# davlee1972/upscale_video

Hardware: AMD Instinct MI355X
Metric: frames/sec 1080p->2x Compact (SRVGGNetCompact per-frame SR hot path) (higher is better)
Workload: dtype f16 operands / f32 accumulate; 1 GPU; 2x_compact_1080p; tile_size=960, frames_per_call=1

## Files before the change

upscale_video_amd/csrc/uva_wino.hip.h:

```cpp
#pragma once
#include <type_traits>

#include "uva_devutil.hip.h"
#include "uva_wino.h"

namespace uva {

constexpr int TW_AROWB = 4 * 2 * 16 * 64;
constexpr int TW_BROWB = 4 * 2 * 15 * 64;
constexpr int TW_AROWS = 6, TW_BROWS = 10;
constexpr int TW_RAWROWB = 34 * 128;
constexpr int TW_RAWSLOTB = 4 * TW_RAWROWB;
constexpr int TW_RAW_PIECES = TW_RAWSLOTB / 1024;
constexpr int TW_ARING = 0;
constexpr int TW_BRING = TW_ARING + TW_AROWS * TW_AROWB;
constexpr int TW_RAW = TW_BRING + TW_BROWS * TW_BROWB;
constexpr int TW_PRM = TW_RAW + 2 * TW_RAWSLOTB;
constexpr int TW_FLAGS_OFF = TW_PRM + 2 * PARAM_LDS + 64;
constexpr int TW_LDS_BYTES = TW_FLAGS_OFF + 16;
static_assert(TW_RAW_PIECES == 17 && TW_RAWSLOTB % 1024 == 0, "raw slot = whole LDS-DMA pieces");
static_assert(TW_LDS_BYTES <= 160 * 1024, "trunkw kernel LDS budget");
static_assert(TW_RAW % 128 == 0 && TW_RAWROWB % 128 == 0, "raw pixel records are 128-byte aligned (the octet XOR flips address bits 4..6)");


__device__ __forceinline__ unsigned tw_piece_const(int i, int wave, int lane)
{
    const int q = (4 * i + wave) * 64 + lane;
    const int r = q / 272, u = q - r * 272;
    const int rec = u >> 3, sl = u & 7;
    const int par = rec >= 17 ? 1 : 0, h = rec - 17 * par;
    return (unsigned)((r << 13) | ((2 * h + par) * 128 + ((sl ^ (h & 7)) << 4)));
}

__device__ __forceinline__ unsigned dpp_row_shl1(unsigned v)
{
    return (unsigned)__builtin_amdgcn_mov_dpp((int)v, 0x101, 0xf, 0xf, true);
}
__device__ __forceinline__ unsigned pk_add_f16(unsigned a, unsigned b)
{
    return __builtin_bit_cast(unsigned, (half2v)(__builtin_bit_cast(half2v, a) + __builtin_bit_cast(half2v, b)));
}

#define TW_PRIO_K 2
#define TW_PRIO_E 0
#define TW_PRIO_KA TW_PRIO_K
#define TW_PRIO_EA TW_PRIO_E
#define TW_PRIO_KB TW_PRIO_K
#define TW_PRIO_EB TW_PRIO_E

#ifdef UVA_INSTRUMENT
#define TW_STAMP(k) do { if (stamp) a.dbg[16 * it + 8 * grp + (k)] = __builtin_amdgcn_s_memtime(); } while (0)
#else
#define TW_STAMP(k) do { } while (0)
#endif

template <int NF, int ACT>
__global__ __launch_bounds__(512, 2) UVA_NO_PK_F32 void trunkw_kernel(TrunkwArgs a)
{
    static_assert(NF == 64, "written for 64 features");
    constexpr int PIXB = 128;
    constexpr int TW_PFF = 12;
    constexpr int TW_PFF_B = 6;
    constexpr int TW_RAW_F0 = 4, TW_RAW_GAP = 12, TW_RAW_STRIDE = 3;
    constexpr int TW_DMA_PIECES = 5;
    constexpr int PFF_A = TW_PFF;

    extern __shared__ __attribute__((aligned(16))) char smem[];
    const unsigned lds0 = lds_offset(smem);
    float* const prm_all = (float*)(smem + TW_PRM);

    const int wave8 = __builtin_amdgcn_readfirstlane(threadIdx.x >> 6);
    const int grp = wave8 >> 2;
    const int wave = wave8 & 3;
    const int lane = threadIdx.x & 63;

#ifdef UVA_INSTRUMENT
    const unsigned long long t_entry = __builtin_amdgcn_s_memtime();
#endif
    const Trunk2Step* const steps = a.steps + (size_t)blockIdx.x * (a.max_steps + TW_PAD_STEPS);
    auto load_a = [&](int g) __attribute__((always_inline)) { return scalar_load16(&steps[g].a); };
    auto load_b = [&](int g) __attribute__((always_inline)) { return scalar_load16(&steps[g].b); };
    const uint4 e_first = load_a(0), e_second = load_a(1);
    const int nsteps = __builtin_amdgcn_readfirstlane(a.nsteps[blockIdx.x]);
    if (nsteps <= 0) return;
#ifdef UVA_INSTRUMENT
    const bool stamp = a.dbg != nullptr && blockIdx.x == 0 && (threadIdx.x & 255) == 0;
    if (stamp && grp == 0) a.dbg[16 * (nsteps + 2)] = t_entry;
#endif

    float prm_b = 0.f, prm_s = 0.f;
    if (wave == 0) {
        prm_b = (grp ? a.bias[1] : a.bias[0])[lane];
        prm_s = (grp ? a.slope[1] : a.slope[0])[lane];
    }
    half8 w[24];
    {
        const half8* wp = (const half8*)(grp ? a.wpk[1] : a.wpk[0]);
#pragma unroll
        for (int i = 0; i < 24; ++i) w[i] = wp[(i * 4 + wave) * 64 + lane];
    }
    unsigned dma_pc2[3];
#pragma unroll
    for (int i = 0; i < 3; ++i)
        dma_pc2[i] = tw_piece_const(2 * i, wave, lane) | (2 * i + 1 < 5 ? tw_piece_const(2 * i + 1, wave, lane) << 16 : 0u);
    auto issue_rows = [&](const uint4 e, int slot, auto i0c, auto i1c) __attribute__((always_inline)) {
        constexpr int I0 = decltype(i0c)::value, I1 = decltype(i1c)::value;
        const unsigned ey = __builtin_amdgcn_readfirstlane(e.y);
        const unsigned lo = __builtin_amdgcn_readfirstlane(e.x), hi = ey & 0xffu;
        const char* base = a.in_act + (((unsigned long long)hi << 32) | lo);
        const int pitch = __builtin_amdgcn_readfirstlane(e.z) & 0xffffff;
        const unsigned fadd = ((ey >> 27) & 1u) ? (unsigned)__builtin_amdgcn_readfirstlane(e.w) : 0u;
#pragma unroll
        for (int i = I0; i < I1; ++i) {
            if (4 * i + wave >= TW_RAW_PIECES) continue;
            const unsigned pc = (dma_pc2[i >> 1] >> (16 * (i & 1))) & 0xffffu;
            unsigned off = __umul24(pc >> 13, (unsigned)pitch) + (pc & 0x1fffu);
            if (fadd) off += (pc & 0x1800u) ? fadd : 0u;
            glds16_s(base, off, lds0 + TW_RAW + slot * TW_RAWSLOTB + (4 * i + wave) * 1024);
        }
    };

    auto vlane_of = [](int l) __attribute__((always_inline)) { const int p_ = l & 15, o_ = l >> 4; return (unsigned)(p_ * 64 + ((o_ ^ ((p_ >> 1) & 3)) << 4)); };

    const unsigned vlane_c = vlane_of(lane);
    const unsigned t_lo = (unsigned)((lane & 15) * PIXB + (((lane >> 4) ^ (lane & 7)) << 4));
    const unsigned t_hi = (unsigned)(((lane & 15) + 1) * PIXB + (((lane >> 4) ^ (((lane & 15) + 1) & 7)) << 4));
    auto transform_row = [&](const char* rrow, int pos) __attribute__((always_inline)) {
        const unsigned a_lo = t_lo, a_hi = t_hi;
        char* const vrow = smem + TW_ARING + pos * TW_AROWB + vlane_c;
        half8 d[2][4];
#pragma unroll
        for (int t = 0; t < 2; ++t) {
            d[t][0] = *(const half8*)(rrow + (a_lo ^ (t ? 64u : 0u)));
            d[t][1] = *(const half8*)(rrow + (a_lo ^ (t ? 64u : 0u)) + 17 * PIXB);
            d[t][2] = *(const half8*)(rrow + (a_hi ^ (t ? 64u : 0u)));
            d[t][3] = *(const half8*)(rrow + (a_hi ^ (t ? 64u : 0u)) + 17 * PIXB);
        }
#pragma unroll
        for (int t = 0; t < 2; ++t) {
            *(half8*)(vrow + 0 * 2048 + t * 1024) = pk_sub(d[t][0], d[t][2]);
            *(half8*)(vrow + 1 * 2048 + t * 1024) = d[t][1] + d[t][2];
            *(half8*)(vrow + 2 * 2048 + t * 1024) = pk_sub(d[t][2], d[t][1]);
            *(half8*)(vrow + 3 * 2048 + t * 1024) = pk_sub(d[t][1], d[t][3]);
        }
    };

    auto transform_half = [&](const char* rrow, int pos, int t) __attribute__((always_inline)) {
        const unsigned a_lo = t_lo ^ (t ? 64u : 0u), a_hi = t_hi ^ (t ? 64u : 0u);
        char* const vrow = smem + TW_ARING + pos * TW_AROWB + vlane_c + t * 1024;
        const half8 d0 = *(const half8*)(rrow + a_lo), d1 = *(const half8*)(rrow + a_lo + 17 * PIXB);
        const half8 d2 = *(const half8*)(rrow + a_hi), d3 = *(const half8*)(rrow + a_hi + 17 * PIXB);
        *(half8*)(vrow + 0 * 2048) = pk_sub(d0, d2);
        *(half8*)(vrow + 1 * 2048) = d1 + d2;
        *(half8*)(vrow + 2 * 2048) = pk_sub(d2, d1);
        *(half8*)(vrow + 3 * 2048) = pk_sub(d1, d3);
    };

    auto transform_rows = [&](int slot, int pos0) __attribute__((always_inline)) {
        int pos = pos0 + wave;
        pos = pos >= TW_AROWS ? pos - TW_AROWS : pos;
        transform_row(smem + TW_RAW + slot * TW_RAWSLOTB + wave * TW_RAWROWB, pos);
    };

    const bool six = (__builtin_amdgcn_readfirstlane(e_first.y) >> 25) & 1u;
    if (grp == 0) {
        issue_rows(e_first, 0, std::integral_constant<int, 0>{}, std::integral_constant<int, 5>{});
        issue_rows(e_second, 1, std::integral_constant<int, 0>{}, std::integral_constant<int, 5>{});
        if (six && wave < 2) {
            const unsigned lo = __builtin_amdgcn_readfirstlane(e_first.x), hi = __builtin_amdgcn_readfirstlane(e_first.y) & 0xffu;
            const int pitch = __builtin_amdgcn_readfirstlane(e_first.z) & 0xffffff;
            const char* base = a.in_act + (((unsigned long long)hi << 32) | lo) - (size_t)(2 - wave) * pitch;
#pragma unroll
            for (int i = 0; i < 5; ++i) {
                int q = i * 64 + lane;
                q = q < 272 ? q : 271;
                const int rec = q >> 3, sl = q & 7, par = rec >= 17 ? 1 : 0, hh = rec - 17 * par;
                glds16_s(base, (unsigned)((2 * hh + par) * 128 + ((sl ^ (hh & 7)) << 4)), lds0 + TW_BRING + wave * 5120 + i * 1024);
            }
        }
#pragma unroll
        for (int i = 0; i < 24; ++i) asm volatile("" : "+v"(w[i]));
        asm volatile("s_waitcnt vmcnt(0)" ::: "memory");
    }
    if (wave == 0) {
        float* prm = prm_all + grp * (PARAM_LDS / 4);
        prm[lane] = prm_b;
        prm[64 + lane] = prm_s;
        prm[128 + lane] = prm_s <= 1.f ? __builtin_inff() : -__builtin_inff();
    }
    group_barrier();
    if (grp == 1) {
        transform_rows(0, 2);
        if (six && wave < 2) transform_row(smem + TW_BRING + wave * 5120, wave);
    }
    group_barrier();

    const float* const bias_lds = prm_all + grp * (PARAM_LDS / 4);
    const float* const prm_lds = bias_lds + 64;
    const f32x4 zero4 = {0.f, 0.f, 0.f, 0.f};
    const f32x4 bias4 = *(const f32x4*)(bias_lds + 16 * wave + 4 * (lane >> 4));
    const f32x4 s4 = *(const f32x4*)(prm_lds + 16 * wave + 4 * (lane >> 4));
    const f32x4 i4 = *(const f32x4*)(prm_lds + 64 + 16 * wave + 4 * (lane >> 4));

    f32x4 acc[4][4];
    [[maybe_unused]] auto prefetch = [&](auto ring_tag, int base_pos, auto& pre) __attribute__((always_inline)) {
        constexpr bool BR = decltype(ring_tag)::value;
        constexpr int ROWB = BR ? TW_BROWB : TW_AROWB;
        constexpr int PFF = BR ? TW_PFF_B : PFF_A;
        static_assert(PFF <= 8, "the fragments read ahead of the barrier are window row 0's");
        const unsigned r0 = vlane_c + (unsigned)((BR ? TW_BRING : TW_ARING) + base_pos * ROWB);
#pragma unroll
        for (int f = 0; f < PFF; ++f) pre[f] = *(const half8*)(smem + r0 + (f & 3) * (ROWB / 4) + ((f >> 2) & 1) * (ROWB / 8));
    };
    auto kloop = [&](auto ring_tag, int base_pos, auto&& slice, auto&& hook, [[maybe_unused]] const auto& pre) __attribute__((always_inline)) {
        constexpr bool BR = decltype(ring_tag)::value;
        constexpr int INR = 0;
        constexpr int ROWB = BR ? TW_BROWB : TW_AROWB, NROWS = BR ? TW_BROWS : TW_AROWS;
        constexpr int JS = ROWB / 4, CS = ROWB / 8;
        constexpr int PFF = BR ? TW_PFF_B : PFF_A;
        constexpr int NFRAG = 48, RQ = PFF + 1;
        unsigned radr[6];
        const unsigned vlane = vlane_c;
#pragma unroll
        for (int R = 0; R < 6; ++R) {
            int pos = base_pos + R;
            pos = pos >= NROWS ? pos - NROWS : pos;
            radr[R] = vlane + (unsigned)((BR ? TW_BRING : TW_ARING) + pos * ROWB);
        }
        auto read_f = [&](int f) __attribute__((always_inline)) -> half8 {
            const int R = f >> 3, ch = (f >> 2) & 1, j = f & 3;
            return *(const half8*)(smem + radr[R] + j * JS + ch * CS);
        };
        half8 bq[RQ];
        __builtin_amdgcn_sched_barrier(0);
#pragma unroll
        for (int f = 0; f < PFF; ++f) {
            if constexpr (BR) bq[f] = pre[f];
            else bq[f] = read_f(f);
        }
        __builtin_amdgcn_sched_barrier(0);
        static_for<NFRAG>([&](auto fc) __attribute__((always_inline)) {
            constexpr int f = decltype(fc)::value;
            if constexpr (f + PFF < NFRAG) bq[(f + PFF) % RQ] = read_f(f + PFF);
            constexpr int R = f >> 3, ch = (f >> 2) & 1, j = f & 3;
            const half8 b = bq[f % RQ];
            static_for<4>([&](auto nc) __attribute__((always_inline)) {
                constexpr int n = decltype(nc)::value, dy = R - n;
                if constexpr (dy >= 0 && dy <= 2) {
                    constexpr bool first = dy == 0 && ch == 0;
                    acc[n][j] = __builtin_amdgcn_mfma_f32_16x16x32_f16(w[(j * 3 + dy) * 2 + ch], b, first ? (j == 1 ? bias4 : zero4) : acc[n][j], 0, 0, 0);
                }
            });
            if constexpr (R >= 3 && R - 3 < INR) slice(std::integral_constant<int, R - 3>{}, std::integral_constant<int, (f & 7)>{});
            hook(fc);
            __builtin_amdgcn_sched_barrier(0);
        });
    };

    struct RowSt {
        f32x2 u, v;
        unsigned x0, x1, y0, y1;
        unsigned t[4], q[8];
    };
    f32x2 neg1 = {-1.f, -1.f};
    asm volatile("" : "+v"(neg1));
    auto fin_sum = [&](RowSt& st, int n, int hh) __attribute__((always_inline)) {
        const f32x2 m0 = {acc[n][0][2 * hh], acc[n][0][2 * hh + 1]}, m1 = {acc[n][1][2 * hh], acc[n][1][2 * hh + 1]};
        const f32x2 m2 = {acc[n][2][2 * hh], acc[n][2][2 * hh + 1]}, m3 = {acc[n][3][2 * hh], acc[n][3][2 * hh + 1]};
        st.u = (m0 + m1) + m2;
        st.v = __builtin_elementwise_fma(m3, neg1, __builtin_elementwise_fma(m2, neg1, m1));
    };
    const half2v s16v[2] = {half2v{(_Float16)s4[0], (_Float16)s4[1]}, half2v{(_Float16)s4[2], (_Float16)s4[3]}};
    auto fin_act = [&](RowSt& st, int hh) __attribute__((always_inline)) {
        if constexpr (ACT != TW_ACT_F32) {
            const half2v hu = __builtin_convertvector(st.u, half2v), hv = __builtin_convertvector(st.v, half2v);
            const half2v mu = hu * s16v[hh], mv = hv * s16v[hh];
            const unsigned xu = __builtin_bit_cast(unsigned, __builtin_elementwise_max(hu, mu));
            const unsigned xv = __builtin_bit_cast(unsigned, __builtin_elementwise_max(hv, mv));
            if (hh == 0) { st.x0 = xu; st.y0 = xv; } else { st.x1 = xu; st.y1 = xv; }
            return;
        }
        const f32x2 sl = {s4[2 * hh], s4[2 * hh + 1]};
        const f32x2 us = st.u * sl, vs = st.v * sl;
        const f32x2 pu = {__builtin_amdgcn_fmed3f(st.u[0], us[0], i4[2 * hh]), __builtin_amdgcn_fmed3f(st.u[1], us[1], i4[2 * hh + 1])};
        const f32x2 pv = {__builtin_amdgcn_fmed3f(st.v[0], vs[0], i4[2 * hh]), __builtin_amdgcn_fmed3f(st.v[1], vs[1], i4[2 * hh + 1])};
        const unsigned xu = __builtin_bit_cast(unsigned, __builtin_convertvector(pu, half2v));
        const unsigned xv = __builtin_bit_cast(unsigned, __builtin_convertvector(pv, half2v));
        if (hh == 0) { st.x0 = xu; st.y0 = xv; } else { st.x1 = xu; st.y1 = xv; }
    };

    const int niter = nsteps + 2;
    __builtin_amdgcn_s_waitcnt(0x0f70);
    RowSt st2[2];
    if (grp == 0) {
        uint4 e_own = load_a(0);
        int a6 = 0;
        int b10 = 0;
        const int cg = lane >> 4, p = lane & 15;
        const int oo = 2 * (wave & 1) + (cg >> 1);
        const unsigned wlane = p < 15 ? (unsigned)(TW_BRING + (2 * (cg & 1)) * (TW_BROWB / 4) + (wave >> 1) * (TW_BROWB / 8) + p * 64 +
                                                    ((oo ^ ((p >> 1) & 3)) << 4))
                                      : (unsigned)(TW_FLAGS_OFF - 64 + 16 * cg);
        const unsigned w64 = (unsigned)(TW_BRING + (wave >> 1) * (TW_BROWB / 8) + p * 64 + ((oo ^ ((p >> 1) & 3)) << 4) + 8 * (cg & 1));
        const unsigned wrow = p < 15 ? (unsigned)TW_BROWB : 0u;
        const unsigned wj = p < 15 ? (unsigned)(TW_BROWB / 4) : 0u;
        half8 pre[PFF_A];
        for (int it = 0; it < niter; ++it) {
            TW_STAMP(0);
            const unsigned ey = __builtin_amdgcn_readfirstlane(e_own.y);
            int rmask = 15, b10w = b10;
            bool in0 = true, in1 = true, edge = false;
            auto set_step = [&](const unsigned eyv, const int b10v) __attribute__((always_inline)) {
                const int c_lo = (eyv >> 12) & 63, c_hi = (eyv >> 18) & 63;
                rmask = (eyv >> 8) & 15;
                const int pm = ((eyv >> 27) & 1u) ? (p & 7) : p;
                in0 = 2 * pm >= c_lo && 2 * pm < c_hi;
                in1 = 2 * pm + 1 >= c_lo && 2 * pm + 1 < c_hi;
                edge = rmask != 15 || c_lo != 0 || c_hi != 32;
                b10w = b10v;
            };
            auto slice = [&](RowSt& st, auto edge_tag, auto nc, auto kc) __attribute__((always_inline)) {
                constexpr int n = decltype(nc)::value, k = decltype(kc)::value;
                if constexpr (k == 0) fin_sum(st, n, 0);
                else if constexpr (k == 1) fin_act(st, 0);
                else if constexpr (k == 2) fin_sum(st, n, 1);
                else if constexpr (k == 3) fin_act(st, 1);
                else if constexpr (k == 4) {
                    if constexpr (decltype(edge_tag)::value) {
                        const bool rin = (rmask >> n) & 1;
                        const unsigned k0 = (rin && in0) ? 0xffffffffu : 0u, k1 = (rin && in1) ? 0xffffffffu : 0u;
                        st.x0 &= k0; st.x1 &= k0;
                        st.y0 &= k1; st.y1 &= k1;
                    }
                    st.t[0] = dpp_row_shl1(st.x0); st.t[1] = dpp_row_shl1(st.x1);
                    st.t[2] = dpp_row_shl1(st.y0); st.t[3] = dpp_row_shl1(st.y1);
                } else if constexpr (k == 5) {
                    st.q[0] = pk_sub_f16(st.x0, st.t[0]); st.q[1] = pk_sub_f16(st.x1, st.t[1]);
                    st.q[2] = pk_add_f16(st.y0, st.t[0]); st.q[3] = pk_add_f16(st.y1, st.t[1]);
                    st.q[4] = pk_sub_f16(st.t[0], st.y0); st.q[5] = pk_sub_f16(st.t[1], st.y1);
                    st.q[6] = pk_sub_f16(st.y0, st.t[2]); st.q[7] = pk_sub_f16(st.y1, st.t[3]);
                } else if constexpr (k == 6) {
                    int pos = b10w + n;
                    pos = pos >= TW_BROWS ? pos - TW_BROWS : pos;
                    if (p < 15) {
                        char* const w0 = smem + w64 + (unsigned)pos * TW_BROWB;
#pragma unroll
                        for (int j = 0; j < 4; ++j) *(uint2*)(w0 + j * (TW_BROWB / 4)) = make_uint2(st.q[2 * j], st.q[2 * j + 1]);
                    }
                } else if constexpr (k == 7) {
                } else if constexpr (k == 8) {
                    const auto s02a = __builtin_amdgcn_permlane16_swap(st.q[0], st.q[4], false, false);
                    const auto s02b = __builtin_amdgcn_permlane16_swap(st.q[1], st.q[5], false, false);
                    const auto s13a = __builtin_amdgcn_permlane16_swap(st.q[2], st.q[6], false, false);
                    const auto s13b = __builtin_amdgcn_permlane16_swap(st.q[3], st.q[7], false, false);
                    st.q[0] = s02a[0]; st.q[1] = s02b[0]; st.q[2] = s02a[1]; st.q[3] = s02b[1];
                    st.q[4] = s13a[0]; st.q[5] = s13b[0]; st.q[6] = s13a[1]; st.q[7] = s13b[1];
                } else {
                    int pos = b10w + n;
                    pos = pos >= TW_BROWS ? pos - TW_BROWS : pos;
                    char* const w0 = smem + wlane + (unsigned)pos * wrow;
                    *(uint4*)w0 = make_uint4(st.q[0], st.q[1], st.q[2], st.q[3]);
                    *(uint4*)(w0 + wj) = make_uint4(st.q[4], st.q[5], st.q[6], st.q[7]);
                }
            };
            set_step(ey, b10);
            if (it < nsteps) {
                __builtin_amdgcn_s_setprio(TW_PRIO_KA);
                auto no_hook = [](auto) __attribute__((always_inline)) {};
                kloop(std::false_type{}, a6, [&](auto nc, auto kc) __attribute__((always_inline)) { slice(st2[0], std::false_type{}, nc, kc); }, no_hook, pre);
                __builtin_amdgcn_s_setprio(TW_PRIO_EA);
            }
            TW_STAMP(1);
            group_barrier();
            TW_STAMP(2);
            if (it < nsteps) {
                auto rest = [&](auto edge_tag) __attribute__((always_inline)) {
                    static_for<2>([&](auto rc) __attribute__((always_inline)) {
                        static_for<8>([&](auto kc) __attribute__((always_inline)) {
                            slice(st2[0], edge_tag, std::integral_constant<int, 2 * decltype(rc)::value>{}, kc);
                            slice(st2[1], edge_tag, std::integral_constant<int, 2 * decltype(rc)::value + 1>{}, kc);
                        });
                    });
                };
                if (edge) rest(std::true_type{}); else rest(std::false_type{});
            }
            e_own = load_a(it + 1 < nsteps ? it + 1 : nsteps - 1);
            TW_STAMP(3);
            a6 = a6 + 4 >= TW_AROWS ? a6 + 4 - TW_AROWS : a6 + 4;
            group_barrier();
            b10 = b10 + 4 >= TW_BROWS ? b10 + 4 - TW_BROWS : b10 + 4;
        }
    } else {
        int a6 = 0, b10 = 0;
        uint4 e_k = make_uint4(0, 0, 0, 0), e_3 = make_uint4(0, 0, 0, 0);
        const int cg = lane >> 4, p = lane & 15;
        const int col = 2 * p + (cg & 1);
        const unsigned olane = (unsigned)(col * PIXB + 32 * wave + 16 * (cg >> 1));
        char* const sink = (char*)a.sink + lane * PIXB;
        const unsigned flip0 = (s4[0] > 1.f ? 0x8000u : 0u) | (s4[1] > 1.f ? 0x80000000u : 0u);
        const unsigned flip1 = (s4[2] > 1.f ? 0x8000u : 0u) | (s4[3] > 1.f ? 0x80000000u : 0u);
        auto make_slice = [&](const uint4 e) __attribute__((always_inline)) {
            const unsigned ey = __builtin_amdgcn_readfirstlane(e.y), lo = __builtin_amdgcn_readfirstlane(e.x);
            const size_t off = ((unsigned long long)(ey & 0xffu) << 32) | lo;
            const int pitch = __builtin_amdgcn_readfirstlane(e.z) & 0xffffff;
            const int vy = (ey >> 8) & 7, vx = (ey >> 11) & 63, v0 = (ey >> 17) & 7;
            const bool fold = (ey >> 25) & 1u;
            const unsigned fadd = fold ? (unsigned)__builtin_amdgcn_readfirstlane(e.w) : 0u;
            char* const obase = a.out_act + off + olane + ((fold && p >= 8) ? fadd : 0u);
            const bool colok = (fold ? (col & 15) : col) < vx;
            return [&, obase, pitch, vy, v0, colok](RowSt& st, auto nc, auto kc) __attribute__((always_inline)) {
                constexpr int n = decltype(nc)::value, k = decltype(kc)::value;
                if constexpr (k == 0) fin_sum(st, n, 0);
                else if constexpr (k == 1) fin_act(st, 0);
                else if constexpr (k == 2) fin_sum(st, n, 1);
                else if constexpr (k == 3) fin_act(st, 1);
                else if constexpr (k == 4) {
                    if constexpr (ACT == TW_ACT_F16_FLIP) {
                        st.x0 ^= flip0; st.y0 ^= flip0;
                        st.x1 ^= flip1; st.y1 ^= flip1;
                    }
                    const auto x = __builtin_amdgcn_permlane16_swap(st.x0, st.y0, false, false);
                    const auto y = __builtin_amdgcn_permlane16_swap(st.x1, st.y1, false, false);
                    st.q[0] = x[0]; st.q[1] = y[0]; st.q[2] = x[1]; st.q[3] = y[1];
                } else if constexpr (k == 5) {
                    char* dst = (n >= v0 && n < vy && colok) ? obase + (size_t)n * pitch : sink;
                    *(uint4*)dst = make_uint4(st.q[0], st.q[1], st.q[2], st.q[3]);
                }
            };
        };
        uint4 e_dma = load_a(2 <= nsteps + TW_PAD_STEPS - 1 ? 2 : nsteps + TW_PAD_STEPS - 1);
        unsigned st_prev = 0;
        for (int it = 0; it < niter; ++it) {
            TW_STAMP(0);
            issue_rows(e_dma, it & 1, std::integral_constant<int, 0>{}, std::integral_constant<int, TW_DMA_PIECES>{});
            e_dma = load_a(it + 3 <= nsteps + TW_PAD_STEPS - 1 ? it + 3 : nsteps + TW_PAD_STEPS - 1);
            const unsigned st_cur = (unsigned)__builtin_amdgcn_readfirstlane((int)(it >= 2 ? (__builtin_amdgcn_readfirstlane(e_3.y) >> 24) & 1u : 0u));
            if (it >= 2 && ((__builtin_amdgcn_readfirstlane(e_3.y) >> 24) & 1u)) {
                auto sl3 = make_slice(e_3);
                static_for<2>([&](auto rc) __attribute__((always_inline)) {
                    static_for<6>([&](auto kc) __attribute__((always_inline)) {
                        sl3(st2[0], std::integral_constant<int, 2 * decltype(rc)::value>{}, kc);
                        sl3(st2[1], std::integral_constant<int, 2 * decltype(rc)::value + 1>{}, kc);
                    });
                });
            }
            e_k = load_b(it >= 1 ? it - 1 : 0);
            const unsigned kact = (it >= 1 && it <= nsteps) ? (__builtin_amdgcn_readfirstlane(e_k.y) >> 24) & 1u : 0u;
            int bp = b10 - 4 - 2;
            bp = bp < 0 ? bp + TW_BROWS : bp;
            half8 pre[TW_PFF_B];
            TW_STAMP(1);
#ifdef UVA_INSTRUMENT
            asm volatile("s_waitcnt vmcnt(0)" ::: "memory");
            st_prev = st_cur;
#else
            {
                constexpr int P0 = TW_DMA_PIECES, P = TW_DMA_PIECES - 1;
                const unsigned nst = st_prev + st_cur;
                if (wave == 0) {
                    if (nst == 2) asm volatile("s_waitcnt vmcnt(%0)" ::"n"(P0 + 8) : "memory");
                    else if (nst == 1) asm volatile("s_waitcnt vmcnt(%0)" ::"n"(P0 + 4) : "memory");
                    else asm volatile("s_waitcnt vmcnt(%0)" ::"n"(P0) : "memory");
                } else {
                    if (nst == 2) asm volatile("s_waitcnt vmcnt(%0)" ::"n"(P + 8) : "memory");
                    else if (nst == 1) asm volatile("s_waitcnt vmcnt(%0)" ::"n"(P + 4) : "memory");
                    else asm volatile("s_waitcnt vmcnt(%0)" ::"n"(P) : "memory");
                }
                st_prev = st_cur;
            }
#endif
            prefetch(std::true_type{}, bp, pre);
            asm volatile("s_barrier" ::: "memory");
            TW_STAMP(2);
            [[maybe_unused]] auto raw_rows = [&]() __attribute__((always_inline)) {
                if (it + 1 < nsteps) {
                    int pos0 = a6 + 4 + 2;
                    pos0 = pos0 >= TW_AROWS ? pos0 - TW_AROWS : pos0;
                    transform_rows((it + 1) & 1, pos0);
                }
            };
            unsigned solo = (unsigned)__builtin_amdgcn_readfirstlane((int)((kact ^ 1u) & (it + 1 < nsteps ? 1u : 0u)));
            asm volatile("" : "+s"(solo));
            if (solo) {
                int pos = a6 + 4 + 2 + wave;
                pos = pos >= 2 * TW_AROWS ? pos - 2 * TW_AROWS : pos >= TW_AROWS ? pos - TW_AROWS : pos;
                const char* const rr = smem + TW_RAW + ((it + 1) & 1) * TW_RAWSLOTB + wave * TW_RAWROWB;
                transform_half(rr, pos, 0);
                __builtin_amdgcn_sched_barrier(0);
                transform_half(rr, pos, 1);
            }
            TW_STAMP(4);
            if (kact) {
                __builtin_amdgcn_s_setprio(TW_PRIO_KB);
                auto slk = make_slice(e_k);
                int rpos = a6 + 4 + 2 + wave;
                rpos = rpos >= 2 * TW_AROWS ? rpos - 2 * TW_AROWS : rpos >= TW_AROWS ? rpos - TW_AROWS : rpos;
                const char* const rrow = smem + TW_RAW + ((it + 1) & 1) * TW_RAWSLOTB + wave * TW_RAWROWB;
                char* const vrow = smem + TW_ARING + rpos * TW_AROWB + vlane_c;
                half8 rd[4];
                auto raw_hook = [&](auto fc) __attribute__((always_inline)) {
                    constexpr int f = decltype(fc)::value;
                    constexpr int H1 = TW_RAW_F0 + TW_RAW_GAP + 3 * TW_RAW_STRIDE + 1;
                    static_assert(H1 + TW_RAW_GAP + 3 * TW_RAW_STRIDE < 48, "the transform ends inside the k-loop");
                    constexpr int t = f >= H1 ? 1 : 0, g = f - (t ? H1 : TW_RAW_F0);
                    const unsigned a_lo = t_lo ^ (t ? 64u : 0u), a_hi = t_hi ^ (t ? 64u : 0u);
                    if constexpr (g == 0) {
                        rd[0] = *(const half8*)(rrow + a_lo); rd[1] = *(const half8*)(rrow + a_lo + 17 * PIXB);
                        rd[2] = *(const half8*)(rrow + a_hi); rd[3] = *(const half8*)(rrow + a_hi + 17 * PIXB);
                    } else if constexpr (g == TW_RAW_GAP) *(half8*)(vrow + 0 * 2048 + t * 1024) = pk_sub(rd[0], rd[2]);
                    else if constexpr (g == TW_RAW_GAP + TW_RAW_STRIDE) *(half8*)(vrow + 3 * 2048 + t * 1024) = pk_sub(rd[1], rd[3]);
                    else if constexpr (g == TW_RAW_GAP + 2 * TW_RAW_STRIDE) *(half8*)(vrow + 1 * 2048 + t * 1024) = rd[1] + rd[2];
                    else if constexpr (g == TW_RAW_GAP + 3 * TW_RAW_STRIDE) *(half8*)(vrow + 2 * 2048 + t * 1024) = pk_sub(rd[2], rd[1]);
                };
                kloop(std::true_type{}, bp, [&](auto nc, auto kc) __attribute__((always_inline)) { slk(st2[0], nc, kc); }, raw_hook, pre);
                __builtin_amdgcn_s_setprio(TW_PRIO_EB);
            }
            e_3 = e_k;
            TW_STAMP(3);
            group_barrier();
            a6 = a6 + 4 >= TW_AROWS ? a6 + 4 - TW_AROWS : a6 + 4;
            b10 = b10 + 4 >= TW_BROWS ? b10 + 4 - TW_BROWS : b10 + 4;
        }
    }
    asm volatile("s_waitcnt vmcnt(0)" ::: "memory");
}

}
```

Measured before the change: 493.4 frames/s.

## Carry partial row accumulators across Winograd k-loop iterations to skip recomputing overlap rows

Adds a carry mode in which the MFMA contributions from the last two input rows of each 6-row window are kept in extra accumulator registers (car) and reused as the starting value for the next iteration's first output rows. The k-loop then reads and multiplies only four new rows per step instead of six, and the prefetch depth and raw-transform schedule shrink to match. Slope, epilogue and DMA-offset constants are rematerialized per iteration instead of being held live, to offset the register pressure of the carry accumulators. The carried state adds a prologue kloop_carry pass and raises accumulator register use, which could hurt occupancy or the scheduling at 2 blocks per CU.

Result: no change. 497.0 frames/s (median of 6 runs) (+0.7%).

```diff
diff --git a/upscale_video_amd/csrc/uva_wino.hip.h b/upscale_video_amd/csrc/uva_wino.hip.h
--- a/upscale_video_amd/csrc/uva_wino.hip.h
+++ b/upscale_video_amd/csrc/uva_wino.hip.h
@@ -59,9 +59,26 @@
 {
     static_assert(NF == 64, "written for 64 features");
     constexpr int PIXB = 128;
-    constexpr int TW_PFF = 12;
-    constexpr int TW_PFF_B = 6;
-    constexpr int TW_RAW_F0 = 4, TW_RAW_GAP = 12, TW_RAW_STRIDE = 3;
+#ifndef TW_CARRY
+#define TW_CARRY 1
+#endif
+#ifndef TW_CARRY_GROUPS
+#define TW_CARRY_GROUPS 3
+#endif
+    constexpr bool CARRY_A = (TW_CARRY != 0) && (TW_CARRY_GROUPS & 1) != 0, CARRY_B = (TW_CARRY != 0) && (TW_CARRY_GROUPS & 2) != 0;
+#ifndef TW_PFF_A_
+#define TW_PFF_A_ (CARRY_A ? 8 : 12)
+#endif
+#ifndef TW_PFF_B_
+#define TW_PFF_B_ (CARRY_B ? 4 : 6)
+#endif
+#ifndef TW_RAW_SCHED
+#define TW_RAW_SCHED 1, 5, 2
+#endif
+    constexpr int TW_PFF = TW_PFF_A_;
+    constexpr int TW_PFF_B = TW_PFF_B_;
+    constexpr int raw_sched_[3] = {TW_RAW_SCHED};
+    constexpr int TW_RAW_F0 = CARRY_B ? raw_sched_[0] : 4, TW_RAW_GAP = CARRY_B ? raw_sched_[1] : 12, TW_RAW_STRIDE = CARRY_B ? raw_sched_[2] : 3;
     constexpr int TW_DMA_PIECES = 5;
     constexpr int PFF_A = TW_PFF;
 
@@ -103,21 +120,30 @@
 #pragma unroll
     for (int i = 0; i < 3; ++i)
         dma_pc2[i] = tw_piece_const(2 * i, wave, lane) | (2 * i + 1 < 5 ? tw_piece_const(2 * i + 1, wave, lane) << 16 : 0u);
-    auto issue_rows = [&](const uint4 e, int slot, auto i0c, auto i1c) __attribute__((always_inline)) {
+    auto piece_of = [&](int i, unsigned& row, unsigned& offs) __attribute__((always_inline)) {
+        const unsigned pc = (dma_pc2[i >> 1] >> (16 * (i & 1))) & 0xffffu;
+        row = pc >> 13;
+        offs = pc & 0x1fffu;
+    };
+    auto issue_rows = [&](const uint4 e, int slot, auto i0c, auto i1c, auto&& piece) __attribute__((always_inline)) {
         constexpr int I0 = decltype(i0c)::value, I1 = decltype(i1c)::value;
         const unsigned ey = __builtin_amdgcn_readfirstlane(e.y);
         const unsigned lo = __builtin_amdgcn_readfirstlane(e.x), hi = ey & 0xffu;
         const char* base = a.in_act + (((unsigned long long)hi << 32) | lo);
         const int pitch = __builtin_amdgcn_readfirstlane(e.z) & 0xffffff;
         const unsigned fadd = ((ey >> 27) & 1u) ? (unsigned)__builtin_amdgcn_readfirstlane(e.w) : 0u;
-#pragma unroll
-        for (int i = I0; i < I1; ++i) {
-            if (4 * i + wave >= TW_RAW_PIECES) continue;
-            const unsigned pc = (dma_pc2[i >> 1] >> (16 * (i & 1))) & 0xffffu;
-            unsigned off = __umul24(pc >> 13, (unsigned)pitch) + (pc & 0x1fffu);
-            if (fadd) off += (pc & 0x1800u) ? fadd : 0u;
-            glds16_s(base, off, lds0 + TW_RAW + slot * TW_RAWSLOTB + (4 * i + wave) * 1024);
-        }
+        auto pieces = [&](auto fold_tag) __attribute__((always_inline)) {
+#pragma unroll
+            for (int i = I0; i < I1; ++i) {
+                if (4 * i + wave >= TW_RAW_PIECES) continue;
+                unsigned row, offs;
+                piece(i, row, offs);
+                unsigned off = __umul24(row, (unsigned)pitch) + offs;
+                if constexpr (decltype(fold_tag)::value) off += (offs & 0x1800u) ? fadd : 0u;
+                glds16_s(base, off, lds0 + TW_RAW + slot * TW_RAWSLOTB + (4 * i + wave) * 1024);
+            }
+        };
+        if (fadd) pieces(std::true_type{}); else pieces(std::false_type{});
     };
 
     auto vlane_of = [](int l) __attribute__((always_inline)) { const int p_ = l & 15, o_ = l >> 4; return (unsigned)(p_ * 64 + ((o_ ^ ((p_ >> 1) & 3)) << 4)); };
@@ -164,8 +190,8 @@
 
     const bool six = (__builtin_amdgcn_readfirstlane(e_first.y) >> 25) & 1u;
     if (grp == 0) {
-        issue_rows(e_first, 0, std::integral_constant<int, 0>{}, std::integral_constant<int, 5>{});
-        issue_rows(e_second, 1, std::integral_constant<int, 0>{}, std::integral_constant<int, 5>{});
+        issue_rows(e_first, 0, std::integral_constant<int, 0>{}, std::integral_constant<int, 5>{}, piece_of);
+        issue_rows(e_second, 1, std::integral_constant<int, 0>{}, std::integral_constant<int, 5>{}, piece_of);
         if (six && wave < 2) {
             const unsigned lo = __builtin_amdgcn_readfirstlane(e_first.x), hi = __builtin_amdgcn_readfirstlane(e_first.y) & 0xffu;
             const int pitch = __builtin_amdgcn_readfirstlane(e_first.z) & 0xffffff;
@@ -199,37 +225,51 @@
     const float* const prm_lds = bias_lds + 64;
     const f32x4 zero4 = {0.f, 0.f, 0.f, 0.f};
     const f32x4 bias4 = *(const f32x4*)(bias_lds + 16 * wave + 4 * (lane >> 4));
-    const f32x4 s4 = *(const f32x4*)(prm_lds + 16 * wave + 4 * (lane >> 4));
-    const f32x4 i4 = *(const f32x4*)(prm_lds + 64 + 16 * wave + 4 * (lane >> 4));
+    f32x4 s4, i4;
+    half2v s16v[2];
+    auto load_slopes = [&](int cg_) __attribute__((always_inline)) {
+        s4 = *(const f32x4*)(prm_lds + 16 * wave + 4 * cg_);
+        if constexpr (ACT == TW_ACT_F32) i4 = *(const f32x4*)(prm_lds + 64 + 16 * wave + 4 * cg_);
+        else {
+            s16v[0] = half2v{(_Float16)s4[0], (_Float16)s4[1]};
+            s16v[1] = half2v{(_Float16)s4[2], (_Float16)s4[3]};
+        }
+    };
 
     f32x4 acc[4][4];
+    [[maybe_unused]] f32x4 car[2][4];
     [[maybe_unused]] auto prefetch = [&](auto ring_tag, int base_pos, auto& pre) __attribute__((always_inline)) {
         constexpr bool BR = decltype(ring_tag)::value;
-        constexpr int ROWB = BR ? TW_BROWB : TW_AROWB;
+        constexpr int ROWB = BR ? TW_BROWB : TW_AROWB, NROWS = BR ? TW_BROWS : TW_AROWS;
         constexpr int PFF = BR ? TW_PFF_B : PFF_A;
-        static_assert(PFF <= 8, "the fragments read ahead of the barrier are window row 0's");
-        const unsigned r0 = vlane_c + (unsigned)((BR ? TW_BRING : TW_ARING) + base_pos * ROWB);
+        constexpr int R0 = (BR ? CARRY_B : CARRY_A) ? 2 : 0;
+        static_assert(PFF <= 8, "the fragments read ahead of the barrier are one window row's");
+        int pos = base_pos + R0;
+        pos = pos >= NROWS ? pos - NROWS : pos;
+        const unsigned r0 = vlane_c + (unsigned)((BR ? TW_BRING : TW_ARING) + pos * ROWB);
 #pragma unroll
         for (int f = 0; f < PFF; ++f) pre[f] = *(const half8*)(smem + r0 + (f & 3) * (ROWB / 4) + ((f >> 2) & 1) * (ROWB / 8));
     };
     auto kloop = [&](auto ring_tag, int base_pos, auto&& slice, auto&& hook, [[maybe_unused]] const auto& pre) __attribute__((always_inline)) {
         constexpr bool BR = decltype(ring_tag)::value;
+        constexpr bool CY = BR ? CARRY_B : CARRY_A;
         constexpr int INR = 0;
         constexpr int ROWB = BR ? TW_BROWB : TW_AROWB, NROWS = BR ? TW_BROWS : TW_AROWS;
         constexpr int JS = ROWB / 4, CS = ROWB / 8;
         constexpr int PFF = BR ? TW_PFF_B : PFF_A;
-        constexpr int NFRAG = 48, RQ = PFF + 1;
-        unsigned radr[6];
+        constexpr int R0 = CY ? 2 : 0;
+        constexpr int NFRAG = (6 - R0) * 8, RQ = PFF + 1;
+        unsigned radr[6 - R0];
         const unsigned vlane = vlane_c;
 #pragma unroll
-        for (int R = 0; R < 6; ++R) {
+        for (int R = R0; R < 6; ++R) {
             int pos = base_pos + R;
             pos = pos >= NROWS ? pos - NROWS : pos;
-            radr[R] = vlane + (unsigned)((BR ? TW_BRING : TW_ARING) + pos * ROWB);
+            radr[R - R0] = vlane + (unsigned)((BR ? TW_BRING : TW_ARING) + pos * ROWB);
         }
         auto read_f = [&](int f) __attribute__((always_inline)) -> half8 {
-            const int R = f >> 3, ch = (f >> 2) & 1, j = f & 3;
-            return *(const half8*)(smem + radr[R] + j * JS + ch * CS);
+            const int Rr = f >> 3, ch = (f >> 2) & 1, j = f & 3;
+            return *(const half8*)(smem + radr[Rr] + j * JS + ch * CS);
         };
         half8 bq[RQ];
         __builtin_amdgcn_sched_barrier(0);
@@ -242,13 +282,26 @@
         static_for<NFRAG>([&](auto fc) __attribute__((always_inline)) {
             constexpr int f = decltype(fc)::value;
             if constexpr (f + PFF < NFRAG) bq[(f + PFF) % RQ] = read_f(f + PFF);
-            constexpr int R = f >> 3, ch = (f >> 2) & 1, j = f & 3;
+            constexpr int R = R0 + (f >> 3), ch = (f >> 2) & 1, j = f & 3;
             const half8 b = bq[f % RQ];
-            static_for<4>([&](auto nc) __attribute__((always_inline)) {
+            static_for<(CY ? 6 : 4)>([&](auto nc) __attribute__((always_inline)) {
                 constexpr int n = decltype(nc)::value, dy = R - n;
                 if constexpr (dy >= 0 && dy <= 2) {
                     constexpr bool first = dy == 0 && ch == 0;
-                    acc[n][j] = __builtin_amdgcn_mfma_f32_16x16x32_f16(w[(j * 3 + dy) * 2 + ch], b, first ? (j == 1 ? bias4 : zero4) : acc[n][j], 0, 0, 0);
+                    const half8 wf = w[(j * 3 + dy) * 2 + ch];
+#ifdef TW_CEIL
+                    if constexpr (n >= 4)
+                        acc[n - 4][j] = __builtin_amdgcn_mfma_f32_16x16x32_f16(wf, b, acc[n - 4][j], 0, 0, 0);
+                    else if constexpr (CY && n < 2 && R == 2 && ch == 0)
+                        acc[n][j] = __builtin_amdgcn_mfma_f32_16x16x32_f16(wf, b, j == 1 ? bias4 : zero4, 0, 0, 0);
+                    else
+#endif
+                    if constexpr (n >= 4)
+                        car[n - 4][j] = __builtin_amdgcn_mfma_f32_16x16x32_f16(wf, b, first ? (j == 1 ? bias4 : zero4) : car[n - 4][j], 0, 0, 0);
+                    else if constexpr (CY && n < 2 && R == 2 && ch == 0)
+                        acc[n][j] = __builtin_amdgcn_mfma_f32_16x16x32_f16(wf, b, car[n][j], 0, 0, 0);
+                    else
+                        acc[n][j] = __builtin_amdgcn_mfma_f32_16x16x32_f16(wf, b, first ? (j == 1 ? bias4 : zero4) : acc[n][j], 0, 0, 0);
                 }
             });
             if constexpr (R >= 3 && R - 3 < INR) slice(std::integral_constant<int, R - 3>{}, std::integral_constant<int, (f & 7)>{});
@@ -256,21 +309,40 @@
             __builtin_amdgcn_sched_barrier(0);
         });
     };
+    [[maybe_unused]] auto kloop_carry = [&](auto ring_tag, int pos4) __attribute__((always_inline)) {
+        constexpr bool BR = decltype(ring_tag)::value;
+        constexpr int ROWB = BR ? TW_BROWB : TW_AROWB, NROWS = BR ? TW_BROWS : TW_AROWS;
+        constexpr int JS = ROWB / 4, CS = ROWB / 8;
+        static_for<2>([&](auto rc) __attribute__((always_inline)) {
+            constexpr int R = 4 + decltype(rc)::value;
+            int pos = pos4 + (R - 4);
+            pos = pos >= NROWS ? pos - NROWS : pos;
+            const unsigned r0 = vlane_c + (unsigned)((BR ? TW_BRING : TW_ARING) + pos * ROWB);
+            half8 bq[8];
+#pragma unroll
+            for (int f = 0; f < 8; ++f) bq[f] = *(const half8*)(smem + r0 + (f & 3) * JS + ((f >> 2) & 1) * CS);
+            static_for<8>([&](auto fc) __attribute__((always_inline)) {
+                constexpr int f = decltype(fc)::value, ch = (f >> 2) & 1, j = f & 3;
+                if constexpr (R == 5) car[0][j] = __builtin_amdgcn_mfma_f32_16x16x32_f16(w[(j * 3 + 1) * 2 + ch], bq[f], car[0][j], 0, 0, 0);
+                f32x4& c = car[R - 4][j];
+                c = __builtin_amdgcn_mfma_f32_16x16x32_f16(w[(j * 3 + 0) * 2 + ch], bq[f], ch == 0 ? (j == 1 ? bias4 : zero4) : c, 0, 0, 0);
+            });
+        });
+    };
 
     struct RowSt {
         f32x2 u, v;
         unsigned x0, x1, y0, y1;
         unsigned t[4], q[8];
     };
-    f32x2 neg1 = {-1.f, -1.f};
-    asm volatile("" : "+v"(neg1));
+    f32x2 neg1;
+    auto make_neg1 = [&]() __attribute__((always_inline)) { neg1 = f32x2{-1.f, -1.f}; asm volatile("" : "+v"(neg1)); };
     auto fin_sum = [&](RowSt& st, int n, int hh) __attribute__((always_inline)) {
         const f32x2 m0 = {acc[n][0][2 * hh], acc[n][0][2 * hh + 1]}, m1 = {acc[n][1][2 * hh], acc[n][1][2 * hh + 1]};
         const f32x2 m2 = {acc[n][2][2 * hh], acc[n][2][2 * hh + 1]}, m3 = {acc[n][3][2 * hh], acc[n][3][2 * hh + 1]};
         st.u = (m0 + m1) + m2;
         st.v = __builtin_elementwise_fma(m3, neg1, __builtin_elementwise_fma(m2, neg1, m1));
     };
-    const half2v s16v[2] = {half2v{(_Float16)s4[0], (_Float16)s4[1]}, half2v{(_Float16)s4[2], (_Float16)s4[3]}};
     auto fin_act = [&](RowSt& st, int hh) __attribute__((always_inline)) {
         if constexpr (ACT != TW_ACT_F32) {
             const half2v hu = __builtin_convertvector(st.u, half2v), hv = __builtin_convertvector(st.v, half2v);
@@ -293,6 +365,11 @@
     __builtin_amdgcn_s_waitcnt(0x0f70);
     RowSt st2[2];
     if (grp == 0) {
+        {
+            int la = lane;
+            asm volatile("" : "+v"(la));
+            load_slopes(la >> 4);
+        }
         uint4 e_own = load_a(0);
         int a6 = 0;
         int b10 = 0;
@@ -305,6 +382,9 @@
         const unsigned wrow = p < 15 ? (unsigned)TW_BROWB : 0u;
         const unsigned wj = p < 15 ? (unsigned)(TW_BROWB / 4) : 0u;
         half8 pre[PFF_A];
+        #ifndef TW_CEIL
+        if constexpr (CARRY_A) kloop_carry(std::false_type{}, 0);
+#endif
         for (int it = 0; it < niter; ++it) {
             TW_STAMP(0);
             const unsigned ey = __builtin_amdgcn_readfirstlane(e_own.y);
@@ -382,6 +462,7 @@
                         });
                     });
                 };
+                make_neg1();
                 if (edge) rest(std::true_type{}); else rest(std::false_type{});
             }
             e_own = load_a(it + 1 < nsteps ? it + 1 : nsteps - 1);
@@ -393,12 +474,23 @@
     } else {
         int a6 = 0, b10 = 0;
         uint4 e_k = make_uint4(0, 0, 0, 0), e_3 = make_uint4(0, 0, 0, 0);
-        const int cg = lane >> 4, p = lane & 15;
-        const int col = 2 * p + (cg & 1);
-        const unsigned olane = (unsigned)(col * PIXB + 32 * wave + 16 * (cg >> 1));
-        char* const sink = (char*)a.sink + lane * PIXB;
-        const unsigned flip0 = (s4[0] > 1.f ? 0x8000u : 0u) | (s4[1] > 1.f ? 0x80000000u : 0u);
-        const unsigned flip1 = (s4[2] > 1.f ? 0x8000u : 0u) | (s4[3] > 1.f ? 0x80000000u : 0u);
+        int p = 0, col = 0;
+        unsigned olane = 0;
+        char* sink = nullptr;
+        unsigned flip0 = 0, flip1 = 0;
+        auto epi_consts = [&]() __attribute__((always_inline)) {
+            int lb = lane;
+            asm volatile("" : "+v"(lb));
+            const int cg = lb >> 4;
+            p = lb & 15;
+            col = 2 * p + (cg & 1);
+            olane = (unsigned)(col * PIXB + 32 * wave + 16 * (cg >> 1));
+            sink = (char*)a.sink + lb * PIXB;
+            load_slopes(cg);
+            flip0 = (s4[0] > 1.f ? 0x8000u : 0u) | (s4[1] > 1.f ? 0x80000000u : 0u);
+            flip1 = (s4[2] > 1.f ? 0x8000u : 0u) | (s4[3] > 1.f ? 0x80000000u : 0u);
+            make_neg1();
+        };
         auto make_slice = [&](const uint4 e) __attribute__((always_inline)) {
             const unsigned ey = __builtin_amdgcn_readfirstlane(e.y), lo = __builtin_amdgcn_readfirstlane(e.x);
             const size_t off = ((unsigned long long)(ey & 0xffu) << 32) | lo;
@@ -430,9 +522,22 @@
         };
         uint4 e_dma = load_a(2 <= nsteps + TW_PAD_STEPS - 1 ? 2 : nsteps + TW_PAD_STEPS - 1);
         unsigned st_prev = 0;
+        unsigned dma_row[5], dma_offs[5];
+        auto dma_unpack = [&]() __attribute__((always_inline)) {
+#pragma unroll
+            for (int i = 0; i < 5; ++i) {
+                unsigned pc2 = dma_pc2[i >> 1];
+                asm volatile("" : "+v"(pc2));
+                const unsigned pc = (pc2 >> (16 * (i & 1))) & 0xffffu;
+                dma_row[i] = pc >> 13;
+                dma_offs[i] = pc & 0x1fffu;
+            }
+        };
+        auto piece_b = [&](int i, unsigned& row, unsigned& offs) __attribute__((always_inline)) { row = dma_row[i]; offs = dma_offs[i]; };
+        dma_unpack();
         for (int it = 0; it < niter; ++it) {
             TW_STAMP(0);
-            issue_rows(e_dma, it & 1, std::integral_constant<int, 0>{}, std::integral_constant<int, TW_DMA_PIECES>{});
+            issue_rows(e_dma, it & 1, std::integral_constant<int, 0>{}, std::integral_constant<int, TW_DMA_PIECES>{}, piece_b);
             e_dma = load_a(it + 3 <= nsteps + TW_PAD_STEPS - 1 ? it + 3 : nsteps + TW_PAD_STEPS - 1);
             const unsigned st_cur = (unsigned)__builtin_amdgcn_readfirstlane((int)(it >= 2 ? (__builtin_amdgcn_readfirstlane(e_3.y) >> 24) & 1u : 0u));
             if (it >= 2 && ((__builtin_amdgcn_readfirstlane(e_3.y) >> 24) & 1u)) {
@@ -490,6 +595,17 @@
                 transform_half(rr, pos, 1);
             }
             TW_STAMP(4);
+#ifndef TW_CEIL
+            if constexpr (CARRY_B) {
+                unsigned cyo = (unsigned)__builtin_amdgcn_readfirstlane((int)((kact ^ 1u) & ((it >= 1 && it <= nsteps) ? 1u : 0u)));
+                asm volatile("" : "+s"(cyo));
+                if (cyo) {
+                    int p4 = bp + 4;
+                    p4 = p4 >= TW_BROWS ? p4 - TW_BROWS : p4;
+                    kloop_carry(std::true_type{}, p4);
+                }
+            }
+#endif
             if (kact) {
                 __builtin_amdgcn_s_setprio(TW_PRIO_KB);
                 auto slk = make_slice(e_k);
@@ -501,7 +617,7 @@
                 auto raw_hook = [&](auto fc) __attribute__((always_inline)) {
                     constexpr int f = decltype(fc)::value;
                     constexpr int H1 = TW_RAW_F0 + TW_RAW_GAP + 3 * TW_RAW_STRIDE + 1;
-                    static_assert(H1 + TW_RAW_GAP + 3 * TW_RAW_STRIDE < 48, "the transform ends inside the k-loop");
+                    static_assert(H1 + TW_RAW_GAP + 3 * TW_RAW_STRIDE < (CARRY_B ? 32 : 48), "the transform ends inside the k-loop");
                     constexpr int t = f >= H1 ? 1 : 0, g = f - (t ? H1 : TW_RAW_F0);
                     const unsigned a_lo = t_lo ^ (t ? 64u : 0u), a_hi = t_hi ^ (t ? 64u : 0u);
                     if constexpr (g == 0) {
@@ -515,6 +631,8 @@
                 kloop(std::true_type{}, bp, [&](auto nc, auto kc) __attribute__((always_inline)) { slk(st2[0], nc, kc); }, raw_hook, pre);
                 __builtin_amdgcn_s_setprio(TW_PRIO_EB);
             }
+            epi_consts();
+            dma_unpack();
             e_3 = e_k;
             TW_STAMP(3);
             group_barrier();
```
